# jayleicn/TVRetrieval

Measured on AMD Instinct MI355X. Metric: queries/sec VCMR over 21.8K-video corpus, higher is better.
Workload: dtype bf16

## Files before the change

include/xmlhip.h:

```cpp
#ifndef XMLHIP_H
#define XMLHIP_H

#include <stddef.h>
#include <stdint.h>

#ifdef __cplusplus
extern "C" {
#endif

typedef void* xml_stream_t;

typedef enum { XML_F32 = 0, XML_BF16 = 1, XML_F16 = 2, XML_F16S = 3 } xml_dtype;
#define XML_F16_UNIT_LOG2 14

typedef enum {
  XML_OK = 0,
  XML_ERR_BAD_ARG = -1,
  XML_ERR_UNSUPPORTED = -2,
  XML_ERR_WORKSPACE = -3,
  XML_ERR_LAUNCH = -4
} xml_status;

int xml_abi_version(void);
const char* xml_build_arch(void);
// ... 2 lines not shown
int xml_pack_weights(const float* src, void* dst, int dt, int64_t n, xml_stream_t stream);
int xml_convert(const void* src, int src_dt, void* dst, int dst_dt, int64_t n, xml_stream_t stream);

size_t xml_linear_ln_relu_pos_workspace_bytes(int64_t rows, int d_in, int hidden, int dt);
int xml_linear_ln_relu_pos(const void* x, int x_dt, const float* ln_in_g, const float* ln_in_b,
                           const void* w, const float* b, const void* pos, const float* ln_pos_g,
                           const float* ln_pos_b, void* y, int64_t rows, int seq_len, int d_in,
                           int hidden, int dt, void* ws, size_t ws_bytes, xml_stream_t stream);


size_t xml_attention_block_workspace_bytes(int64_t n, int seq_len, int hidden, int dt);
int xml_attention_block(const void* x, const float* key_mask, const void* wqkv, const float* bqkv,
                        const void* wo, const float* bo, const float* ln_g, const float* ln_b,
                        void* y, int64_t n, int seq_len, int hidden, int n_heads, int dt, void* ws,
                        size_t ws_bytes, xml_stream_t stream);

int xml_attention_core(const void* q, int ldq, const void* k, int ldk, const void* v, int ldv, const float* q_mask,
                       const float* k_mask, void* out, int64_t n, int lq, int lk, int hidden, int n_heads, int dt,
                       xml_stream_t stream);

int xml_pack_plan(const float* mask, int64_t n, int lq, int32_t* cu_seqlens, int32_t* src_row, int32_t* status,
                  xml_stream_t stream);
size_t xml_linear_ln_relu_pos_packed_workspace_bytes(int64_t rows, int d_in, int hidden, int dt);
int xml_linear_ln_relu_pos_packed(const void* x, int x_dt, const int32_t* src_row, int lq, const float* ln_in_g,
                                  const float* ln_in_b, const void* w, const float* b, const void* pos,
                                  const float* ln_pos_g, const float* ln_pos_b, void* y, int64_t rows, int d_in,
                                  int hidden, int dt, void* ws, size_t ws_bytes, xml_stream_t stream);
size_t xml_attention_block_varlen_workspace_bytes(int64_t rows, int hidden, int dt);
int xml_attention_block_varlen(const void* x, const int32_t* cu_seqlens, const void* wqkv, const float* bqkv,
                               const void* wo, const float* bo, const float* ln_g, const float* ln_b, void* y,
// ... 263 lines not shown
```

tvretrieval_amd/_lib.py:

```python
import ctypes
import os
from ctypes import c_char_p, c_float, c_int, c_int32, c_int64, c_size_t, c_void_p

_HERE = os.path.dirname(os.path.abspath(__file__))
LIB_PATH = os.environ.get("XMLHIP_LIB") or os.path.join(_HERE, "csrc", "libxmlhip.so")

XML_F32 = 0
XML_BF16 = 1
XML_F16 = 2
XML_F16S = 3

ABI_VERSION = 6


class XmlHipError(RuntimeError):
    pass


class ConvseDesc(ctypes.Structure):
    _fields_ = [(n, c_int) for n in
                ("nq", "nv", "kpairs", "lpad", "l_ref", "hidden", "n_mod", "merged", "ksize", "softmax", "dt")]


SIGNATURES = {
    "xml_abi_version": (c_int, []),
    "xml_build_arch": (c_char_p, []),
    "xml_status_string": (c_char_p, [c_int]),
    "xml_pack_weights": (c_int, [c_void_p, c_void_p, c_int, c_int64, c_void_p]),
    "xml_convert": (c_int, [c_void_p, c_int, c_void_p, c_int, c_int64, c_void_p]),
    "xml_linear_ln_relu_pos_workspace_bytes": (c_size_t, [c_int64, c_int, c_int, c_int]),
    "xml_linear_ln_relu_pos": (c_int, [c_void_p, c_int, c_void_p, c_void_p, c_void_p, c_void_p, c_void_p, c_void_p,
                                       c_void_p, c_void_p, c_int64, c_int, c_int, c_int, c_int, c_void_p, c_size_t,
                                       c_void_p]),
    "xml_attention_block_workspace_bytes": (c_size_t, [c_int64, c_int, c_int, c_int]),
    "xml_attention_block": (c_int, [c_void_p, c_void_p, c_void_p, c_void_p, c_void_p, c_void_p, c_void_p, c_void_p,
                                    c_void_p, c_int64, c_int, c_int, c_int, c_int, c_void_p, c_size_t, c_void_p]),
    "xml_pack_plan": (c_int, [c_void_p, c_int64, c_int, c_void_p, c_void_p, c_void_p, c_void_p]),
    "xml_linear_ln_relu_pos_packed_workspace_bytes": (c_size_t, [c_int64, c_int, c_int, c_int]),
    "xml_linear_ln_relu_pos_packed": (c_int, [c_void_p, c_int, c_void_p, c_int, c_void_p, c_void_p, c_void_p, c_void_p,
                                              c_void_p, c_void_p, c_void_p, c_void_p, c_int64, c_int, c_int, c_int,
                                              c_void_p, c_size_t, c_void_p]),
    "xml_attention_block_varlen_workspace_bytes": (c_size_t, [c_int64, c_int, c_int]),
    "xml_attention_block_varlen": (c_int, [c_void_p, c_void_p, c_void_p, c_void_p, c_void_p, c_void_p, c_void_p, c_void_p,
                                           c_void_p, c_int64, c_int64, c_int, c_int, c_int, c_int, c_void_p, c_size_t,
                                           c_void_p]),
    "xml_modular_pool_varlen": (c_int, [c_void_p, c_void_p, c_void_p, c_void_p, c_int64, c_int, c_int, c_int, c_int,
                                        c_void_p]),
    "xml_cross_attention_workspace_bytes": (c_size_t, [c_int64, c_int, c_int, c_int, c_int]),
    "xml_cross_attention": (c_int, [c_void_p, c_void_p, c_void_p, c_void_p, c_void_p, c_void_p, c_void_p, c_void_p,
                                    c_void_p, c_void_p, c_void_p, c_int64, c_int, c_int, c_int, c_int, c_int,
                                    c_void_p, c_size_t, c_void_p]),
# ... 198 lines not shown
```

tvretrieval_amd/csrc/attention.hip:

```cpp
#include <type_traits>

#include "gemm.h"
#include "internal.h"

template <typename T> struct ChunkOf { static constexpr int elems = 64 / (int)sizeof(T); };

typedef short xml_v4s __attribute__((ext_vector_type(4)));
__device__ __forceinline__ uint2 lds_read_tr16(const char* p) {
  const xml_v4s r = __builtin_amdgcn_ds_read_tr16_b64_v4i16((__attribute__((address_space(3))) xml_v4s*)p);
  return __builtin_bit_cast(uint2, r);
}

#ifdef XML_DEBUG_VARIANTS
__device__ unsigned long long g_attn_probe[16];
extern "C" int xml_debug_read_attn_probe(unsigned long long* host_out) {
  return hipMemcpyFromSymbol(host_out, HIP_SYMBOL(g_attn_probe), sizeof(unsigned long long) * 16) == hipSuccess ? 0 : -4;
}
#define XML_ATTN_PROBE(i) do { if (abl == 8 && blockIdx.x == 1 && blockIdx.y == 300 && threadIdx.x == 64) g_attn_probe[i] = __builtin_amdgcn_s_memtime(); } while (0)
#else
#define XML_ATTN_PROBE(i) do { } while (0)
#endif

template <typename T, typename OutT, int DH>
__global__ __launch_bounds__(256) void attention_core_kernel(const T* __restrict__ Q, int ldq,
// ... 523 lines not shown
  if (!q || !k || !v || !k_mask || !out) return XML_ERR_BAD_ARG;
  if (dt != XML_F32 && dt != XML_BF16) return XML_ERR_BAD_ARG;
  if (ldq < hidden || ldk < hidden || ldv < hidden || (ldq | ldk | ldv | hidden) % 8) return XML_ERR_UNSUPPORTED;
  return xmli_attention_core(q, ldq, k, ldk, v, ldv, q_mask, k_mask, out, 0, n, lq, lk, hidden, n_heads, dt,
                             (hipStream_t)stream);
}

extern "C" size_t xml_attention_block_workspace_bytes(int64_t n, int seq_len, int hidden, int dt) {
  const size_t rows = (size_t)n * seq_len;
  const size_t pre = align_up(rows * hidden * 4, 256);
  const size_t lnw = xmli_gemm_ln_eligible((int64_t)rows, hidden, hidden, dt) ? xmli_gemm_ln_workspace_bytes((int64_t)rows, hidden) : 0;
  return align_up(rows * 3 * hidden * dt_size(dt), 256) + align_up(rows * hidden * dt_size(dt), 256) +
         (pre > lnw ? pre : lnw) + xmli_gemm_split_ws_bytes((int64_t)rows, hidden, dt);
}

extern "C" int xml_attention_block(const void* x, const float* key_mask, const void* wqkv, const float* bqkv,
                                   const void* wo, const float* bo, const float* ln_g, const float* ln_b, void* y,
                                   int64_t n, int seq_len, int hidden, int n_heads, int dt, void* ws, size_t ws_bytes,
                                   xml_stream_t stream) {
  XML_ENTER();
  if (!x || !key_mask || !wqkv || !bqkv || !wo || !bo || !ln_g || !ln_b || !y || !ws) return XML_ERR_BAD_ARG;
  if (n <= 0 || seq_len <= 0 || !xmli_model_dt_ok(dt)) return XML_ERR_BAD_ARG;
  if (seq_len > 128 || hidden % 8) return XML_ERR_UNSUPPORTED;
  if (ws_bytes < xml_attention_block_workspace_bytes(n, seq_len, hidden, dt)) return XML_ERR_WORKSPACE;
  hipStream_t st = (hipStream_t)stream;
  const int64_t rows = n * seq_len;
  const int adt = xmli_act_dt(dt);
  char* qkv = (char*)ws;
  char* att = qkv + align_up((size_t)rows * 3 * hidden * dt_size(dt), 256);
  char* pre = att + align_up((size_t)rows * hidden * dt_size(dt), 256);
  char* sws = dt == XML_F16S ? (char*)ws + xml_attention_block_workspace_bytes(n, seq_len, hidden, dt) -
                                   xmli_gemm_split_ws_bytes(rows, hidden, dt) : nullptr;
  int rc = xmli_gemm(x, wqkv, bqkv, nullptr, qkv, rows, 3 * hidden, hidden, 0, 0, 1, 0, dt, st, sws);
  if (rc) return rc;
  const size_t es = dt_size(dt);
  rc = xmli_attention_core(qkv, 3 * hidden, qkv + (size_t)hidden * es, 3 * hidden, qkv + (size_t)2 * hidden * es,
                           3 * hidden, nullptr, key_mask, att, 0, n, seq_len, seq_len, hidden, n_heads, adt, st);
  if (rc) return rc;
  if (xmli_gemm_ln_eligible(rows, hidden, hidden, dt) && y != x &&
      xmli_gemm_ln(att, wo, bo, x, ln_g, ln_b, y, rows, hidden, hidden, 0,  2, 1, dt, pre, st) == XML_OK)
    return XML_OK;
  rc = xmli_gemm(att, wo, bo, x, pre, rows, hidden, hidden, 0,  2, 1,  1, dt, st, sws);
  if (rc) return rc;
  return xmli_gemm_ln_tail((const float*)pre, ln_g, ln_b, y, rows, hidden, dt, st);
}

template <typename T, int DH>
static int launch_attn_varlen(const char* qkv, int hidden, const int32_t* cu, void* att, int64_t n, int max_len,
                              int n_heads, int dt, hipStream_t st) {
  const size_t lds_s = attn_small_lds_bytes(max_len, DH, dt);
  if (lds_s > 160 * 1024) return XML_ERR_UNSUPPORTED;
  if (lds_s > 64 * 1024 && !xml_lds_attr_once<attention_core_small_kernel<T, T, DH>>(160 * 1024)) return XML_ERR_LAUNCH;
  const int64_t units = n * n_heads;
  const T* q = (const T*)qkv;
  hipLaunchKernelGGL((attention_core_small_kernel<T, T, DH>), dim3((unsigned)((units + 3) / 4)), dim3(256), lds_s, st, q,
                     3 * hidden, q + hidden, 3 * hidden, q + 2 * hidden, 3 * hidden, (const float*)nullptr,
                     (const float*)nullptr, (T*)att, hidden, max_len, max_len, n_heads, units, sqrtf((float)DH), cu);
  XML_CHECK_LAUNCH();
  return XML_OK;
// ... 430 lines not shown
```

tvretrieval_amd/csrc/gemm256p.hip:

```cpp
#include <type_traits>

#include "common.h"
#include "internal.h"

struct G256pArgs {
  const void* A;
  const void* W;
  const float* bias;
  const void* addend;
  void* out;
  int64_t M, n_tiles;
  int N, K, relu, add_mode, seq_len, tn;
  float* ln_scratch;
  const float* ln_g;
  const float* ln_b;
  float ln_eps;
  int probe;
};

__device__ __forceinline__ void g256p_dma_pair(uint32_t v0, uint32_t v1, const char* sb, uint32_t lds_dst) {
  asm volatile(
      "s_mov_b32 m0, %2\n\ts_nop 0\n\tglobal_load_lds_dwordx4 %0, %3\n\t"
      "s_add_u32 m0, m0, 0x400\n\ts_nop 0\n\tglobal_load_lds_dwordx4 %1, %3"
      :
      : "v"(v0), "v"(v1), "s"(lds_dst), "s"(sb)
      : "memory", "scc");
}
__device__ __forceinline__ void g256p_dma_quad(uint32_t v0, uint32_t v1, uint32_t v2, uint32_t v3, const char* sb,
                                               uint32_t lds_dst) {
  asm volatile(
      "s_mov_b32 m0, %4\n\ts_nop 0\n\tglobal_load_lds_dwordx4 %0, %5\n\t"
      "s_add_u32 m0, m0, 0x400\n\ts_nop 0\n\tglobal_load_lds_dwordx4 %1, %5\n\t"
// ... 36 lines not shown
__device__ __forceinline__ uint4 dpp_u4(const uint4& v) {
  uint4 r;
  r.x = (uint32_t)__builtin_amdgcn_update_dpp(0, (int)v.x, CTRL, 0xf, 0xf, false);
  r.y = (uint32_t)__builtin_amdgcn_update_dpp(0, (int)v.y, CTRL, 0xf, 0xf, false);
  r.z = (uint32_t)__builtin_amdgcn_update_dpp(0, (int)v.z, CTRL, 0xf, 0xf, false);
  r.w = (uint32_t)__builtin_amdgcn_update_dpp(0, (int)v.w, CTRL, 0xf, 0xf, false);
  return r;
}
__device__ __forceinline__ int g256p_lane_now() {
  int l;
  asm volatile("v_mbcnt_lo_u32_b32 %0, -1, 0\n\tv_mbcnt_hi_u32_b32 %0, -1, %0" : "=v"(l));
  return l;
}
__device__ __forceinline__ int g256p_swz(int row) { return (0x78 >> (((row >> 2) & 3) << 1)) & 3; }

template <typename T, typename OutT, typename AddT, bool LNE = false, bool DIRECT = true>
__global__ __launch_bounds__(512) void gemm256p_kernel(G256pArgs a) {
  static_assert(!LNE || DIRECT, "the LayerNorm epilogue works on the DIRECT accumulator layout");
  constexpr int ROWB = 64;
  constexpr int OPER_BYTES = 256 * ROWB;
  constexpr int SLOT_BYTES = 2 * OPER_BYTES;
  constexpr int NSLOT = 4;
  constexpr int RING_BYTES = NSLOT * SLOT_BYTES;
  extern __shared__ __attribute__((aligned(16))) char smem[];

  const int tid = threadIdx.x, lane = tid & 63;
  const int wave = __builtin_amdgcn_readfirstlane(tid >> 6);
  const int wm = wave >> 1, wn = wave & 1;
  const int grp = wave >> 2;
  const int fr = lane & 15, fg = lane >> 4;
  const int xcd = blockIdx.x & 7, loc = blockIdx.x >> 3;
  const int k_bytes = a.K * (int)sizeof(T);
  const int n_slices = k_bytes / ROWB;
// ... 177 lines not shown
    };
    slice_step(faA, faB, std::true_type{});
    slice_step(faB, faA, std::false_type{});
    for (int s2 = 2; s2 < n_slices; s2 += 2) {
      slice_step(faA, faB, std::false_type{});
      slice_step(faB, faA, std::false_type{});
    }

    { const unsigned long long t = G256P_T(); pr[0] += t - pt; pt = t; }
    {
      int64_t mt; int nt;
      tile_mt_nt(c_k, mt, nt);
      const int64_t m0 = mt * 256;
      const int n0 = nt * 256;
      const uint32_t m0_mod = a.add_mode == 1 ? (uint32_t)(m0 % a.seq_len) : 0u;
      const int lane_e = g256p_lane_now();
      const int fr_e = lane_e & 15, fg_e = lane_e >> 4;
      const int tid_e = wave * 64 + lane_e;
      float* patch = reinterpret_cast<float*>(smem + RING_BYTES) + wave * 1024;
      constexpr bool F32O = sizeof(OutT) == 4;
      const int orow = lane_e >> 4;
      const int oc0 = (lane_e & 15) * (F32O ? 4 : 8);
      const int oc1 = F32O ? oc0 + 64 : oc0 + 4;
      const int nc0 = n0 + wn * 128 + oc0, nc1 = n0 + wn * 128 + oc1;
      const bool ok0 = nc0 + 4 <= N, ok1 = nc1 + 4 <= N;
      constexpr int GC = PAIRED ? 8 : 4;
      constexpr int NGRP = 128 / (4 * GC);
      static_assert(GC * sizeof(AddT) <= 16, "addend group wider than one 16-byte load");
      int gcol[DIRECT ? NGRP : 1];
      bool gok[DIRECT ? NGRP : 1];
      int pcol[DIRECT ? NGRP / 2 : 1];
      auto store_rows = [&](int m4, auto& v, int dcol = 0) {
        uint4 pk[NGRP];
#pragma unroll
        for (int q = 0; q < NGRP; ++q) pk[q] = pack16<OutT>(v[q]);
        const bool odd = (fr_e & 1) != 0;
        const int64_t m_even = m0 + wm * 64 + m4 * 16 + (fr_e & ~1);
#pragma unroll
        for (int pq = 0; pq < NGRP / 2; ++pq) {
          const uint4 dn = dpp_u4<0x111>(pk[2 * pq + 1]);
          const uint4 up = dpp_u4<0x101>(pk[2 * pq]);
          const uint4 own_e = pk[2 * pq], own_o = pk[2 * pq + 1];
          const uint4 d_even = make_uint4(odd ? dn.x : own_e.x, odd ? dn.y : own_e.y, odd ? dn.z : own_e.z, odd ? dn.w : own_e.w);
          const uint4 d_odd = make_uint4(odd ? own_o.x : up.x, odd ? own_o.y : up.y, odd ? own_o.z : up.z, odd ? own_o.w : up.w);
          const int col = pcol[pq] + dcol;
          if (col + GC <= N) {
            if (!(a.probe & 8)) {
              typedef unsigned int g_u4 __attribute__((ext_vector_type(4)));
              if (m_even < M && !(a.probe & 4)) __builtin_nontemporal_store(g_u4{d_even.x, d_even.y, d_even.z, d_even.w}, reinterpret_cast<g_u4*>(out + m_even * N + col));
              if (m_even + 1 < M && !(a.probe & 4)) __builtin_nontemporal_store(g_u4{d_odd.x, d_odd.y, d_odd.z, d_odd.w}, reinterpret_cast<g_u4*>(out + (m_even + 1) * N + col));
            } else {
              if (m_even < M && !(a.probe & 4)) st_global16(out + m_even * N + col, d_even);
              if (m_even + 1 < M && !(a.probe & 4)) st_global16(out + (m_even + 1) * N + col, d_odd);
            }
          }
        }
      };
      if constexpr (DIRECT) {
#pragma unroll
        for (int q = 0; q < NGRP; ++q) {
          gcol[q] = n0 + wn * 128 + q * (4 * GC) + fg_e * GC;
          gok[q] = gcol[q] + GC <= N;
        }
#pragma unroll
        for (int pq = 0; pq < NGRP / 2; ++pq) pcol[pq] = n0 + wn * 128 + pq * (8 * GC) + (fr_e & 1) * (4 * GC) + fg_e * GC;
        {
          float4 b4 = make_float4(0.f, 0.f, 0.f, 0.f);
          const int bc = n0 + wn * 128 + (lane_e & 31) * 4;
// ... 255 lines not shown
#ifdef XML_DEBUG_VARIANTS
  if ((a.probe & 1) && blockIdx.x == 0 && lane == 0) {
    pr[5] = __builtin_amdgcn_s_memtime() - pr_t0;
    pr[7] = __builtin_amdgcn_s_memrealtime() - pr_r0;
    for (int i = 0; i < 8; ++i) g_g256p_probe[wave * 8 + i] = pr[i];
    for (int i = 0; i < 64; ++i) g_g256p_steps[wave * 64 + i] = sp[i];
  }
#endif
  };
  if (grp) run(std::true_type{});
  else run(std::false_type{});
  asm volatile("s_waitcnt vmcnt(0)" ::: "memory");
  __builtin_amdgcn_s_barrier();
}

template <typename T, typename OutT, typename AddT, bool LNE = false, bool DIRECT = true>
static int launch_gemm256p(const void* A, const void* W, const float* bias, const void* addend, void* out, int64_t M,
                           int N, int K, int relu, int add_mode, int seq_len, hipStream_t st, const float* ln_g = nullptr,
                           const float* ln_b = nullptr, void* ln_ws = nullptr) {
  G256pArgs a;
  a.A = A; a.W = W; a.bias = bias; a.addend = addend; a.out = out;
  a.M = M; a.N = N; a.K = K; a.relu = relu; a.add_mode = add_mode; a.seq_len = seq_len;
  a.tn = cdiv(N, 256);
  a.n_tiles = (int64_t)cdiv(M, 256) * a.tn;
  a.ln_scratch = (float*)ln_ws; a.ln_g = ln_g; a.ln_b = ln_b; a.ln_eps = 1e-5f;
  a.probe = g_q2c_ablation == 9 ? 1 : g_q2c_ablation == 21 ? 2 : g_q2c_ablation == 22 ? 4 : g_q2c_ablation == 23 ? 6 : g_q2c_ablation == 24 ? 8 : 0;
  const int lds = 4 * 2 * 256 * 64 + 8 * 4096;
#ifdef XML_DEBUG_VARIANTS
  if (!LNE && DIRECT && g_gemm_variant == 3)
    return launch_gemm256p<T, OutT, AddT, false, false>(A, W, bias, addend, out, M, N, K, relu, add_mode, seq_len, st);
#endif
  auto kern = gemm256p_kernel<T, OutT, AddT, LNE, DIRECT>;
  if (!xml_lds_attr_once<gemm256p_kernel<T, OutT, AddT, LNE, DIRECT>>(lds)) return XML_ERR_LAUNCH;
  hipLaunchKernelGGL(kern, dim3(256), dim3(512), lds, st, a);
  XML_CHECK_LAUNCH();
  return XML_OK;
}

static constexpr int64_t LN_FUSED_MIN_ROWS = 2048;

bool xmli_gemm_ln_eligible(int64_t M, int N, int K, int dt) {
  if (dt != XML_F32 && dt != XML_BF16) return false;
  const size_t kb = (size_t)K * dt_size(dt);
  return kb % 128 == 0 && kb >= 256 && N % 256 == 0 && N / 256 <= 3 && M >= LN_FUSED_MIN_ROWS;
}
size_t xmli_gemm_ln_workspace_bytes(int64_t M, int N) {
  (void)M;
  return align_up((size_t)256 * (size_t)(N / 256 > 1 ? N / 256 - 1 : 0) * 256 * 256 * 4 + 256, 256);
}
int xmli_gemm_ln(const void* A, const void* W, const float* bias, const void* addend, const float* ln_g, const float* ln_b,
                 void* y, int64_t M, int N, int K, int relu, int add_mode, int seq_len, int dt, void* ln_ws,
                 hipStream_t st) {
  if (!ln_ws) return XML_ERR_WORKSPACE;
  if (dt == XML_F32)
    return launch_gemm256p<float, float, float, true>(A, W, bias, addend, y, M, N, K, relu, add_mode, seq_len, st, ln_g,
                                                      ln_b, ln_ws);
  return launch_gemm256p<bf16_t, bf16_t, bf16_t, true>(A, W, bias, addend, y, M, N, K, relu, add_mode, seq_len, st, ln_g,
                                                        ln_b, ln_ws);
}

template <typename OutT, int TN>
__global__ __launch_bounds__(64) void ln_lne_order_kernel(const float* __restrict__ pre, const float* __restrict__ ln_g,
                                                           const float* __restrict__ ln_b, OutT* __restrict__ y,
                                                           int64_t rows, int N, float ln_eps) {
#pragma clang fp contract(off)
  constexpr int GC = sizeof(OutT) == 2 ? 8 : 4;
  constexpr int NGRP = 128 / (4 * GC);
  constexpr int LPR = TN == 1 ? 8 : TN == 2 ? 16 : 32;
  const int lane = threadIdx.x & 63;
  const int sub = lane & (LPR - 1);
  const int base = lane - sub;
  const int64_t row = ((int64_t)blockIdx.x * 64 + threadIdx.x) / LPR;
  if (row >= rows || sub >= 8 * TN) return;
  const int seg = sub >> 2, fg = sub & 3;
  const int c0 = (seg >> 1) * 256 + (seg & 1) * 128 + fg * GC;
  const float* pr = pre + row * N;
  float v[NGRP][GC], gv[NGRP][GC], bv[NGRP][GC];
#pragma unroll
  for (int q = 0; q < NGRP; ++q)
#pragma unroll
    for (int e = 0; e < GC; e += 4) {
      const float4 f = *reinterpret_cast<const float4*>(pr + c0 + q * (4 * GC) + e);
      const float4 g4 = *reinterpret_cast<const float4*>(ln_g + c0 + q * (4 * GC) + e);
      const float4 b4 = *reinterpret_cast<const float4*>(ln_b + c0 + q * (4 * GC) + e);
      v[q][e] = f.x; v[q][e + 1] = f.y; v[q][e + 2] = f.z; v[q][e + 3] = f.w;
      gv[q][e] = g4.x; gv[q][e + 1] = g4.y; gv[q][e + 2] = g4.z; gv[q][e + 3] = g4.w;
      bv[q][e] = b4.x; bv[q][e + 1] = b4.y; bv[q][e + 2] = b4.z; bv[q][e + 3] = b4.w;
    }
#pragma unroll
  for (int q = 0; q < NGRP; ++q)
#pragma unroll
// ... 29 lines not shown
  float m2 = 0.f;
#pragma unroll
  for (int t = 0; t < TN; ++t) {
    const float d0 = __builtin_fmaf(pv[t].x, 1.0f / 128.0f, -mean), d1 = __builtin_fmaf(pv[t].z, 1.0f / 128.0f, -mean);
    float u = __builtin_fmaf(d0, 128.0f * d0, pv[t].y);
    u = pv[t].w + u;
    u = __builtin_fmaf(d1, 128.0f * d1, u);
    m2 = u + m2;
  }
  const float rstd = 1.0f / sqrtf(m2 / (float)N + ln_eps);
#pragma unroll
  for (int q = 0; q < NGRP; ++q) {
    float o[GC];
#pragma unroll
    for (int e = 0; e < GC; ++e) o[e] = __builtin_fmaf((v[q][e] - mean) * rstd, gv[q][e], bv[q][e]);
    st_global16(y + row * N + c0 + q * (4 * GC), pack16<OutT>(o));
  }
}

int xmli_gemm_ln_tail(const float* pre, const float* ln_g, const float* ln_b, void* y, int64_t M, int N, int dt,
                      hipStream_t st) {
  const int tn = N / 256;
  if ((dt != XML_F32 && dt != XML_BF16) || N % 256 || tn < 1 || tn > 3 || M <= 0)
    return xmli_add_layernorm(pre, XML_F32, nullptr, ln_g, ln_b, y, M, N, N, xmli_act_dt(dt), st);
  const int lpr = tn == 1 ? 8 : tn == 2 ? 16 : 32;
  const dim3 grid((unsigned)cdiv(M * lpr, (int64_t)64)), blk(64);
#define XML_LNT(OT, TN)                                                                                                 \
  hipLaunchKernelGGL((ln_lne_order_kernel<OT, TN>), grid, blk, 0, st, pre, ln_g, ln_b, (OT*)y, M, N, 1e-5f)
  if (dt == XML_F32) {
    if (tn == 1) XML_LNT(float, 1); else if (tn == 2) XML_LNT(float, 2); else XML_LNT(float, 3);
  } else {
    if (tn == 1) XML_LNT(bf16_t, 1); else if (tn == 2) XML_LNT(bf16_t, 2); else XML_LNT(bf16_t, 3);
  }
#undef XML_LNT
  XML_CHECK_LAUNCH();
  return XML_OK;
}

bool xmli_gemm256p_eligible(int64_t M, int N, int K, int dt) {
  const size_t kb = (size_t)K * dt_size(dt);
  return kb % 128 == 0 && kb >= 256 && N >= 128 && N % 8 == 0 && (int64_t)cdiv(M, 256) * cdiv(N, 256) >= 3072;
}

// ... 9 lines not shown
```

tvretrieval_amd/csrc/internal.h:

```cpp
#pragma once
#include "common.h"

int xmli_gemm(const void* A, const void* W, const float* bias, const void* addend, void* out, int64_t M, int N,
              int K, int relu, int add_mode, int seq_len, int out_f32, int dt, hipStream_t st, void* split_ws = nullptr);
size_t xmli_gemm_split_ws_bytes(int64_t M, int K, int dt);
static inline int xmli_act_dt(int dt) { return dt == XML_F16S ? XML_F32 : dt; }
static inline bool xmli_model_dt_ok(int dt) { return dt == XML_F32 || dt == XML_BF16 || dt == XML_F16S; }
bool xmli_gemm_ln_eligible(int64_t M, int N, int K, int dt);
size_t xmli_gemm_ln_workspace_bytes(int64_t M, int N);
int xmli_gemm_ln(const void* A, const void* W, const float* bias, const void* addend, const float* ln_g, const float* ln_b,
                 void* y, int64_t M, int N, int K, int relu, int add_mode, int seq_len, int dt, void* ln_ws,
                 hipStream_t st);
int xmli_gemm_ln_tail(const float* pre, const float* ln_g, const float* ln_b, void* y, int64_t M, int N, int dt,
                      hipStream_t st);
int xmli_add_layernorm(const void* a, int a_dt, const void* b, const float* g, const float* beta, void* y,
                       int64_t rows, int d, int ld_out, int dt, hipStream_t st);
int xmli_attention_core(const void* q, int ldq, const void* k, int ldk, const void* v, int ldv,
                        const float* q_mask, const float* k_mask, void* out, int out_f32, int64_t n, int lq, int lk,
                        int hidden, int n_heads, int dt, hipStream_t st);
int xmli_modular_pool_bwd_vec(const void* enc, const float* mask, const float* w_m, const void* dout, void* denc, float* dw_m,
                              int64_t n, int lq, int hidden, int n_mod, int dt, hipStream_t st);
```

tvretrieval_amd/inference.py:

```python
import numpy as np
import torch

from . import ops as hip_ops


def _round_up(x, m):
    return (x + m - 1) // m * m


class CorpusIndex(object):

    def __init__(self, modalities, feat1n, feat2, mask, l_ref, video_offset=0, n_total=None):
        self.modalities = list(modalities)
        self.feat1n, self.feat2, self.mask = feat1n, feat2, mask
        self.l_ref = int(l_ref)
        self.lpad = int(feat2[self.modalities[0]].shape[1])
        self.n_videos = int(feat2[self.modalities[0]].shape[0])
        self.video_offset = int(video_offset)
        self.n_total = int(n_total if n_total is not None else self.n_videos)
        self.feat2_all = self.mask_all = None
        self.exact = None
        self.vlen = self.vlen_all = None
        self.ragged = False

# ... 98 lines not shown
        self.n_videos, self.l_ref, self.lpad = int(n_videos), int(l_ref), index_lpad(l_ref, model, ops)
        self.f1 = {m: torch.zeros((self.n_videos, self.lpad, h), dtype=dt, device=dev) for m in mods}
        self.f2 = {m: torch.zeros((self.n_videos, self.lpad, h), dtype=dt, device=dev) for m in mods}
        self.mk = {m: torch.zeros((self.n_videos, self.lpad), dtype=torch.float32, device=dev) for m in mods}
        self.tiles = {}
        if tiles and hasattr(ops, "q2c_tiled_numel") and self.lpad == 128 and dt in (torch.float32, torch.bfloat16):
            n = ops.q2c_tiled_numel(self.n_videos * self.lpad, h, dt)
            if n:
                self.tiles = {m: torch.zeros(n, dtype=dt, device=dev) for m in mods}

    def nbytes(self):
        return sum(t.numel() * t.element_size() for d in (self.f1, self.f2, self.mk, self.tiles) for t in d.values())


def build_corpus_index(model, context_batches, ops=hip_ops, keep_raw=False, video_offset=0, n_total=None,
                        l_ref=None, n_videos=None, exact_filter=False, storage=None):
    mods = [n for n, u in (("video", model.use_video), ("sub", model.use_sub)) if u]
    if storage is not None:
        assert l_ref is None or int(l_ref) == storage.l_ref
        assert n_videos is None or int(n_videos) == storage.n_videos
        l_ref, n_videos = storage.l_ref, storage.n_videos
    if n_videos is not None and l_ref is not None:
        return _build_corpus_index_prealloc(model, context_batches, ops, keep_raw, video_offset, n_total, int(l_ref),
                                            int(n_videos), mods, exact_filter, storage)
    parts = {m: dict(f1=[], f2=[], mk=[]) for m in mods}
    for video_feat, video_mask, sub_feat, sub_mask in context_batches:
        v1, v2, s1, s2 = model.encode_context(video_feat, video_mask, sub_feat, sub_mask)
        if "video" in parts:
            parts["video"]["f1"].append(v1), parts["video"]["f2"].append(v2), parts["video"]["mk"].append(video_mask.float())
        if "sub" in parts:
            parts["sub"]["f1"].append(s1), parts["sub"]["f2"].append(s2), parts["sub"]["mk"].append(sub_mask.float())
    batch_max = max(t.shape[1] for t in parts[mods[0]]["f2"])
    l_ref = batch_max if l_ref is None else int(l_ref)
    assert l_ref >= batch_max
    lpad = index_lpad(l_ref, model, ops)

    def cat(tensors):
        n = sum(t.shape[0] for t in tensors)
        out = tensors[0].new_zeros((n, lpad) + tuple(tensors[0].shape[2:]))
# ... 22 lines not shown
            raw[m] = f1
    idx = CorpusIndex(mods, feat1n, feat2, mask, l_ref, video_offset, n_total)
    if getattr(ops, "RAGGED_ROWS", False):
        idx.set_valid_lengths()
    idx.raw_feat1 = raw
    if exact_filter:
        idx.exact = _make_exact_filter(ex_f32, ex_ec, exact_mode_of(model, ops))
    return idx


def _make_exact_filter(ex_f32, ex_ec, mode):
    return ExactFilter(ex_f32, ex_ec, n_candidates=128 if (mode == "f16s" and EXACT_F16S_FILTER == "f16") else 256, mode=mode)


def _build_corpus_index_prealloc(model, context_batches, ops, keep_raw, video_offset, n_total, l_ref, n_videos, mods,
                                 exact_filter=False, storage=None):
    lpad = index_lpad(l_ref, model, ops)
    f1, f2, mk = {}, {}, {}
    if storage is not None:
        f1, f2, mk = dict(storage.f1), dict(storage.f2), dict(storage.mk)
    r = 0
    for video_feat, video_mask, sub_feat, sub_mask in context_batches:
        outs = [None, None, None, None]
        direct = bool(f1) and getattr(ops, "ENCODE_INTO_INDEX", False)
        if direct:
            for i, (m, feat) in enumerate((("video", video_feat), ("sub", sub_feat))):
                b = feat.shape[0] if feat is not None else 0
                if m in mods and feat is not None and feat.shape[1] == lpad and r + b <= n_videos:
                    outs[2 * i], outs[2 * i + 1] = f1[m][r:r + b], f2[m][r:r + b]
                elif m in mods:
                    direct = False
        if direct:
            v1, v2, s1, s2 = model.encode_context(video_feat, video_mask, sub_feat, sub_mask, outs=tuple(outs))
        else:
            v1, v2, s1, s2 = model.encode_context(video_feat, video_mask, sub_feat, sub_mask)
        for m, a1, a2, am in (("video", v1, v2, video_mask), ("sub", s1, s2, sub_mask)):
            if m not in mods:
                continue
            if m not in f1:
                f1[m] = a1.new_zeros((n_videos, lpad, a1.shape[2]))
                f2[m] = a2.new_zeros((n_videos, lpad, a2.shape[2]))
                mk[m] = torch.zeros((n_videos, lpad), dtype=torch.float32, device=a1.device)
            b, lb = a1.shape[0], a1.shape[1]
            assert r + b <= n_videos and lb <= l_ref
            if not direct:
                f1[m][r:r + b, :lb] = a1
                f2[m][r:r + b, :lb] = a2
            mk[m][r:r + b, :lb] = am.float()
        r += v1.shape[0] if v1 is not None else s1.shape[0]
    assert r == n_videos, "n_videos=%d but the batches held %d" % (n_videos, r)
    plan = ops.q2c_pack_plan([mk[m] for m in mods]) if (hasattr(ops, "q2c_pack_plan") and lpad == 128) else None
    feat1n, raw, ex_f32, ex_ec = {}, {}, {}, {}
    for m in mods:
        if exact_filter:
            feat1n[m], ex_f32[m], ex_ec[m] = _exact_filter_operands(f1[m], mk[m], plan, ops, exact_mode_of(model, ops))
            if exact_mode_of(model, ops) == "f16s":
                f2[m] = ops.split_f16_rows(f2[m])
        else:
            tile_buf = storage.tiles.get(m) if (storage is not None and plan is None) else None
            kw = dict(out=tile_buf) if tile_buf is not None else {}
            feat1n[m] = ops.pack_q2c_corpus(f1[m], mk[m], plan, normalize=True, **kw) if hasattr(ops, "pack_q2c_corpus") \
# ... 1148 lines not shown
```

tvretrieval_amd/ops.py:

```python
import collections
import ctypes

import os

import numpy as np

import torch

from . import _lib
from ._lib import XML_BF16, XML_F32, ConvseDesc, check

class _SplitF16(object):

    def __repr__(self):
        return "tvretrieval_amd.ops.F16S"


F16S = _SplitF16()
_DT = {torch.float32: XML_F32, torch.bfloat16: XML_BF16, torch.float16: _lib.XML_F16, F16S: _lib.XML_F16S}
F16_UNIT_LOG2 = 14


def act_dtype(dtype):
    return torch.float32 if dtype is F16S else dtype
# ... 125 lines not shown
    if v < 0:
        check(v, what)
    return v


ENCODE_INTO_INDEX = True


def _req_w(w, name, x):
    _req(w, name)
    if not (w.dtype == x.dtype or (w.dtype is F16S and x.dtype == torch.float32)):
        raise _lib.XmlHipError("%s: weight dtype %s does not go with activations of dtype %s" % (name, w.dtype, x.dtype))
    return w


def attention_block(x, key_mask, wqkv, bqkv, wo, bo, ln_g, ln_b, n_heads, out=None):
    _req(x, "x"); _req(key_mask, "key_mask", torch.float32); _req_w(wqkv, "wqkv", x); _req_w(wo, "wo", x)
    for t, nm in ((bqkv, "bqkv"), (bo, "bo"), (ln_g, "ln_g"), (ln_b, "ln_b")):
        _req(t, nm, torch.float32)
    n, seq_len, hidden = x.shape
    lib = _lib.load()
    dt = dt_of(wqkv)
    if out is None:
        y = torch.empty_like(x)
    else:
        _req(out, "out", x.dtype)
        assert out.shape == x.shape and out.data_ptr() != x.data_ptr()
        y = out
    ws = _workspace(lib.xml_attention_block_workspace_bytes(n, seq_len, hidden, dt), x.device)
    check(lib.xml_attention_block(_p(x), _p(key_mask), _p(wqkv), _p(bqkv), _p(wo), _p(bo), _p(ln_g), _p(ln_b), _p(y),
                                  n, seq_len, hidden, n_heads, dt, _p(ws), ws.numel(), _stream()),
          "xml_attention_block")
    return y


def attention_core(q, k, v, q_mask, k_mask, n_heads):
    _req(q, "q"); _req(k, "k", q.dtype); _req(v, "v", q.dtype); _req(k_mask, "k_mask", torch.float32)
    if q_mask is not None:
        _req(q_mask, "q_mask", torch.float32)
    n, lq, hidden = q.shape
    lk = k.shape[1]
    assert k.shape == v.shape and k.shape[0] == n and k.shape[2] == hidden
    out = torch.empty((n, lq, hidden), dtype=q.dtype, device=q.device)
    check(_lib.load().xml_attention_core(_p(q), hidden, _p(k), hidden, _p(v), hidden, _p(q_mask), _p(k_mask), _p(out), n, lq,
                                         lk, hidden, int(n_heads), dt_of(q), _stream()), "xml_attention_core")
    return out

# ... 889 lines not shown
```

Before: 146,700.

## Write attention-block output directly into padded corpus index via strided rows

Adds a sequence-strided output mode to the attention block, covering both the GEMM+LayerNorm epilogue kernel and the LN tail kernel, so encoder output can land straight in a slice of the preallocated padded index tensors even when the batch length is shorter than the index padding. The Python index builder now infers n_videos up front, preallocates the index (using torch.empty when every batch already matches the padding), and passes strided views into encode_context. This is meant to remove the intermediate output tensors and the copy into the index, plus the zero-fill. The cost is extra per-row address arithmetic (divide/modulo) in the epilogue and more complex control flow in the builder.

After: 146,700 (median of 2 runs). Within noise of the previous version (-0.0%).

```diff
diff --git a/include/xmlhip.h b/include/xmlhip.h
--- a/include/xmlhip.h
+++ b/include/xmlhip.h
@@ -40,6 +40,11 @@
                         const void* wo, const float* bo, const float* ln_g, const float* ln_b,
                         void* y, int64_t n, int seq_len, int hidden, int n_heads, int dt, void* ws,
                         size_t ws_bytes, xml_stream_t stream);
+int xml_attention_block_to_ok(int hidden, int dt);
+int xml_attention_block_to(const void* x, const float* key_mask, const void* wqkv, const float* bqkv,
+                           const void* wo, const float* bo, const float* ln_g, const float* ln_b,
+                           void* y, int64_t y_seq_stride, int64_t n, int seq_len, int hidden, int n_heads, int dt,
+                           void* ws, size_t ws_bytes, xml_stream_t stream);
 
 int xml_attention_core(const void* q, int ldq, const void* k, int ldk, const void* v, int ldv, const float* q_mask,
                        const float* k_mask, void* out, int64_t n, int lq, int lk, int hidden, int n_heads, int dt,
diff --git a/tvretrieval_amd/_lib.py b/tvretrieval_amd/_lib.py
--- a/tvretrieval_amd/_lib.py
+++ b/tvretrieval_amd/_lib.py
@@ -35,6 +35,9 @@
     "xml_attention_block_workspace_bytes": (c_size_t, [c_int64, c_int, c_int, c_int]),
     "xml_attention_block": (c_int, [c_void_p, c_void_p, c_void_p, c_void_p, c_void_p, c_void_p, c_void_p, c_void_p,
                                     c_void_p, c_int64, c_int, c_int, c_int, c_int, c_void_p, c_size_t, c_void_p]),
+    "xml_attention_block_to_ok": (c_int, [c_int, c_int]),
+    "xml_attention_block_to": (c_int, [c_void_p, c_void_p, c_void_p, c_void_p, c_void_p, c_void_p, c_void_p, c_void_p,
+                                       c_void_p, c_int64, c_int64, c_int, c_int, c_int, c_int, c_void_p, c_size_t, c_void_p]),
     "xml_pack_plan": (c_int, [c_void_p, c_int64, c_int, c_void_p, c_void_p, c_void_p, c_void_p]),
     "xml_linear_ln_relu_pos_packed_workspace_bytes": (c_size_t, [c_int64, c_int, c_int, c_int]),
     "xml_linear_ln_relu_pos_packed": (c_int, [c_void_p, c_int, c_void_p, c_int, c_void_p, c_void_p, c_void_p, c_void_p,
diff --git a/tvretrieval_amd/csrc/attention.hip b/tvretrieval_amd/csrc/attention.hip
--- a/tvretrieval_amd/csrc/attention.hip
+++ b/tvretrieval_amd/csrc/attention.hip
@@ -561,14 +561,17 @@
          (pre > lnw ? pre : lnw) + xmli_gemm_split_ws_bytes((int64_t)rows, hidden, dt);
 }
 
-extern "C" int xml_attention_block(const void* x, const float* key_mask, const void* wqkv, const float* bqkv,
-                                   const void* wo, const float* bo, const float* ln_g, const float* ln_b, void* y,
-                                   int64_t n, int seq_len, int hidden, int n_heads, int dt, void* ws, size_t ws_bytes,
-                                   xml_stream_t stream) {
-  XML_ENTER();
+static int attention_block_impl(const void* x, const float* key_mask, const void* wqkv, const float* bqkv,
+                                const void* wo, const float* bo, const float* ln_g, const float* ln_b, void* y,
+                                int64_t y_seq_stride, int64_t n, int seq_len, int hidden, int n_heads, int dt, void* ws,
+                                size_t ws_bytes, xml_stream_t stream) {
   if (!x || !key_mask || !wqkv || !bqkv || !wo || !bo || !ln_g || !ln_b || !y || !ws) return XML_ERR_BAD_ARG;
   if (n <= 0 || seq_len <= 0 || !xmli_model_dt_ok(dt)) return XML_ERR_BAD_ARG;
   if (seq_len > 128 || hidden % 8) return XML_ERR_UNSUPPORTED;
+  if (y_seq_stride < (int64_t)seq_len * hidden) return XML_ERR_BAD_ARG;
+  const int y_seq_len = y_seq_stride == (int64_t)seq_len * hidden ? 0 : seq_len;
+  if (y_seq_len && !xml_attention_block_to_ok(hidden, dt)) return XML_ERR_UNSUPPORTED;
+  if (y_seq_len && (y_seq_stride % 8 || y == x)) return XML_ERR_UNSUPPORTED;
   if (ws_bytes < xml_attention_block_workspace_bytes(n, seq_len, hidden, dt)) return XML_ERR_WORKSPACE;
   hipStream_t st = (hipStream_t)stream;
   const int64_t rows = n * seq_len;
@@ -585,11 +588,34 @@
                            3 * hidden, nullptr, key_mask, att, 0, n, seq_len, seq_len, hidden, n_heads, adt, st);
   if (rc) return rc;
   if (xmli_gemm_ln_eligible(rows, hidden, hidden, dt) && y != x &&
-      xmli_gemm_ln(att, wo, bo, x, ln_g, ln_b, y, rows, hidden, hidden, 0,  2, 1, dt, pre, st) == XML_OK)
+      xmli_gemm_ln(att, wo, bo, x, ln_g, ln_b, y, rows, hidden, hidden, 0,  2, 1, dt, pre, st, y_seq_stride,
+                   y_seq_len) == XML_OK)
     return XML_OK;
   rc = xmli_gemm(att, wo, bo, x, pre, rows, hidden, hidden, 0,  2, 1,  1, dt, st, sws);
   if (rc) return rc;
-  return xmli_gemm_ln_tail((const float*)pre, ln_g, ln_b, y, rows, hidden, dt, st);
+  return xmli_gemm_ln_tail((const float*)pre, ln_g, ln_b, y, rows, hidden, dt, st, y_seq_stride, y_seq_len);
+}
+
+extern "C" int xml_attention_block(const void* x, const float* key_mask, const void* wqkv, const float* bqkv,
+                                   const void* wo, const float* bo, const float* ln_g, const float* ln_b, void* y,
+                                   int64_t n, int seq_len, int hidden, int n_heads, int dt, void* ws, size_t ws_bytes,
+                                   xml_stream_t stream) {
+  XML_ENTER();
+  return attention_block_impl(x, key_mask, wqkv, bqkv, wo, bo, ln_g, ln_b, y, (int64_t)seq_len * hidden, n, seq_len, hidden,
+                              n_heads, dt, ws, ws_bytes, stream);
+}
+
+extern "C" int xml_attention_block_to_ok(int hidden, int dt) {
+  return (dt == XML_F32 || dt == XML_BF16) && hidden > 0 && hidden % 256 == 0 && hidden / 256 <= 3;
+}
+
+extern "C" int xml_attention_block_to(const void* x, const float* key_mask, const void* wqkv, const float* bqkv,
+                                      const void* wo, const float* bo, const float* ln_g, const float* ln_b, void* y,
+                                      int64_t y_seq_stride, int64_t n, int seq_len, int hidden, int n_heads, int dt, void* ws,
+                                      size_t ws_bytes, xml_stream_t stream) {
+  XML_ENTER();
+  return attention_block_impl(x, key_mask, wqkv, bqkv, wo, bo, ln_g, ln_b, y, y_seq_stride, n, seq_len, hidden, n_heads, dt,
+                              ws, ws_bytes, stream);
 }
 
 template <typename T, int DH>
diff --git a/tvretrieval_amd/csrc/gemm256p.hip b/tvretrieval_amd/csrc/gemm256p.hip
--- a/tvretrieval_amd/csrc/gemm256p.hip
+++ b/tvretrieval_amd/csrc/gemm256p.hip
@@ -16,6 +16,8 @@
   const float* ln_b;
   float ln_eps;
   int probe;
+  int64_t out_seq_stride;
+  int out_seq_len;
 };
 
 __device__ __forceinline__ void g256p_dma_pair(uint32_t v0, uint32_t v1, const char* sb, uint32_t lds_dst) {
@@ -82,9 +84,10 @@
 }
 __device__ __forceinline__ int g256p_swz(int row) { return (0x78 >> (((row >> 2) & 3) << 1)) & 3; }
 
-template <typename T, typename OutT, typename AddT, bool LNE = false, bool DIRECT = true>
+template <typename T, typename OutT, typename AddT, bool LNE = false, bool DIRECT = true, bool OSEQ = false>
 __global__ __launch_bounds__(512) void gemm256p_kernel(G256pArgs a) {
   static_assert(!LNE || DIRECT, "the LayerNorm epilogue works on the DIRECT accumulator layout");
+  static_assert(!OSEQ || LNE, "sequence-strided output rows: LayerNorm-epilogue kernels only");
   constexpr int ROWB = 64;
   constexpr int OPER_BYTES = 256 * ROWB;
   constexpr int SLOT_BYTES = 2 * OPER_BYTES;
@@ -292,6 +295,12 @@
       const int64_t m0 = mt * 256;
       const int n0 = nt * 256;
       const uint32_t m0_mod = a.add_mode == 1 ? (uint32_t)(m0 % a.seq_len) : 0u;
+      int64_t o_seq0 = 0;
+      uint32_t o_row0 = 0;
+      if constexpr (OSEQ) {
+        o_seq0 = m0 / a.out_seq_len;
+        o_row0 = (uint32_t)(m0 - o_seq0 * a.out_seq_len);
+      }
       const int lane_e = g256p_lane_now();
       const int fr_e = lane_e & 15, fg_e = lane_e >> 4;
       const int tid_e = wave * 64 + lane_e;
@@ -314,6 +323,15 @@
         for (int q = 0; q < NGRP; ++q) pk[q] = pack16<OutT>(v[q]);
         const bool odd = (fr_e & 1) != 0;
         const int64_t m_even = m0 + wm * 64 + m4 * 16 + (fr_e & ~1);
+        OutT* o_even = nullptr;
+        OutT* o_odd = nullptr;
+        if constexpr (OSEQ) {
+          const uint32_t sl = (uint32_t)a.out_seq_len;
+          const uint32_t u0 = o_row0 + (uint32_t)(wm * 64 + m4 * 16 + (fr_e & ~1)), u1 = u0 + 1;
+          const uint32_t d0 = u0 / sl, d1 = u1 / sl;
+          o_even = out + (o_seq0 + d0) * a.out_seq_stride + (int64_t)(u0 - d0 * sl) * N;
+          o_odd = out + (o_seq0 + d1) * a.out_seq_stride + (int64_t)(u1 - d1 * sl) * N;
+        }
 #pragma unroll
         for (int pq = 0; pq < NGRP / 2; ++pq) {
           const uint4 dn = dpp_u4<0x111>(pk[2 * pq + 1]);
@@ -325,11 +343,11 @@
           if (col + GC <= N) {
             if (!(a.probe & 8)) {
               typedef unsigned int g_u4 __attribute__((ext_vector_type(4)));
-              if (m_even < M && !(a.probe & 4)) __builtin_nontemporal_store(g_u4{d_even.x, d_even.y, d_even.z, d_even.w}, reinterpret_cast<g_u4*>(out + m_even * N + col));
-              if (m_even + 1 < M && !(a.probe & 4)) __builtin_nontemporal_store(g_u4{d_odd.x, d_odd.y, d_odd.z, d_odd.w}, reinterpret_cast<g_u4*>(out + (m_even + 1) * N + col));
+              if (m_even < M && !(a.probe & 4)) __builtin_nontemporal_store(g_u4{d_even.x, d_even.y, d_even.z, d_even.w}, reinterpret_cast<g_u4*>(OSEQ ? o_even + col : out + m_even * N + col));
+              if (m_even + 1 < M && !(a.probe & 4)) __builtin_nontemporal_store(g_u4{d_odd.x, d_odd.y, d_odd.z, d_odd.w}, reinterpret_cast<g_u4*>(OSEQ ? o_odd + col : out + (m_even + 1) * N + col));
             } else {
-              if (m_even < M && !(a.probe & 4)) st_global16(out + m_even * N + col, d_even);
-              if (m_even + 1 < M && !(a.probe & 4)) st_global16(out + (m_even + 1) * N + col, d_odd);
+              if (m_even < M && !(a.probe & 4)) st_global16(OSEQ ? o_even + col : out + m_even * N + col, d_even);
+              if (m_even + 1 < M && !(a.probe & 4)) st_global16(OSEQ ? o_odd + col : out + (m_even + 1) * N + col, d_odd);
             }
           }
         }
@@ -615,24 +633,26 @@
   __builtin_amdgcn_s_barrier();
 }
 
-template <typename T, typename OutT, typename AddT, bool LNE = false, bool DIRECT = true>
+template <typename T, typename OutT, typename AddT, bool LNE = false, bool DIRECT = true, bool OSEQ = false>
 static int launch_gemm256p(const void* A, const void* W, const float* bias, const void* addend, void* out, int64_t M,
                            int N, int K, int relu, int add_mode, int seq_len, hipStream_t st, const float* ln_g = nullptr,
-                           const float* ln_b = nullptr, void* ln_ws = nullptr) {
+                           const float* ln_b = nullptr, void* ln_ws = nullptr, int64_t out_seq_stride = 0,
+                           int out_seq_len = 0) {
   G256pArgs a;
   a.A = A; a.W = W; a.bias = bias; a.addend = addend; a.out = out;
   a.M = M; a.N = N; a.K = K; a.relu = relu; a.add_mode = add_mode; a.seq_len = seq_len;
   a.tn = cdiv(N, 256);
   a.n_tiles = (int64_t)cdiv(M, 256) * a.tn;
   a.ln_scratch = (float*)ln_ws; a.ln_g = ln_g; a.ln_b = ln_b; a.ln_eps = 1e-5f;
+  a.out_seq_stride = out_seq_stride; a.out_seq_len = out_seq_len;
   a.probe = g_q2c_ablation == 9 ? 1 : g_q2c_ablation == 21 ? 2 : g_q2c_ablation == 22 ? 4 : g_q2c_ablation == 23 ? 6 : g_q2c_ablation == 24 ? 8 : 0;
   const int lds = 4 * 2 * 256 * 64 + 8 * 4096;
 #ifdef XML_DEBUG_VARIANTS
   if (!LNE && DIRECT && g_gemm_variant == 3)
     return launch_gemm256p<T, OutT, AddT, false, false>(A, W, bias, addend, out, M, N, K, relu, add_mode, seq_len, st);
 #endif
-  auto kern = gemm256p_kernel<T, OutT, AddT, LNE, DIRECT>;
-  if (!xml_lds_attr_once<gemm256p_kernel<T, OutT, AddT, LNE, DIRECT>>(lds)) return XML_ERR_LAUNCH;
+  auto kern = gemm256p_kernel<T, OutT, AddT, LNE, DIRECT, OSEQ>;
+  if (!xml_lds_attr_once<gemm256p_kernel<T, OutT, AddT, LNE, DIRECT, OSEQ>>(lds)) return XML_ERR_LAUNCH;
   hipLaunchKernelGGL(kern, dim3(256), dim3(512), lds, st, a);
   XML_CHECK_LAUNCH();
   return XML_OK;
@@ -651,8 +671,16 @@
 }
 int xmli_gemm_ln(const void* A, const void* W, const float* bias, const void* addend, const float* ln_g, const float* ln_b,
                  void* y, int64_t M, int N, int K, int relu, int add_mode, int seq_len, int dt, void* ln_ws,
-                 hipStream_t st) {
+                 hipStream_t st, int64_t y_seq_stride, int y_seq_len) {
   if (!ln_ws) return XML_ERR_WORKSPACE;
+  if (y_seq_len > 0 && y_seq_stride != (int64_t)y_seq_len * N) {
+    if (y_seq_stride < (int64_t)y_seq_len * N) return XML_ERR_BAD_ARG;
+    if (dt == XML_F32)
+      return launch_gemm256p<float, float, float, true, true, true>(A, W, bias, addend, y, M, N, K, relu, add_mode, seq_len,
+                                                                    st, ln_g, ln_b, ln_ws, y_seq_stride, y_seq_len);
+    return launch_gemm256p<bf16_t, bf16_t, bf16_t, true, true, true>(A, W, bias, addend, y, M, N, K, relu, add_mode, seq_len,
+                                                                      st, ln_g, ln_b, ln_ws, y_seq_stride, y_seq_len);
+  }
   if (dt == XML_F32)
     return launch_gemm256p<float, float, float, true>(A, W, bias, addend, y, M, N, K, relu, add_mode, seq_len, st, ln_g,
                                                       ln_b, ln_ws);
@@ -660,10 +688,11 @@
                                                         ln_b, ln_ws);
 }
 
-template <typename OutT, int TN>
+template <typename OutT, int TN, bool OSEQ = false>
 __global__ __launch_bounds__(64) void ln_lne_order_kernel(const float* __restrict__ pre, const float* __restrict__ ln_g,
                                                            const float* __restrict__ ln_b, OutT* __restrict__ y,
-                                                           int64_t rows, int N, float ln_eps) {
+                                                           int64_t rows, int N, float ln_eps, int64_t y_seq_stride,
+                                                           int y_seq_len) {
 #pragma clang fp contract(off)
   constexpr int GC = sizeof(OutT) == 2 ? 8 : 4;
   constexpr int NGRP = 128 / (4 * GC);
@@ -676,6 +705,8 @@
   const int seg = sub >> 2, fg = sub & 3;
   const int c0 = (seg >> 1) * 256 + (seg & 1) * 128 + fg * GC;
   const float* pr = pre + row * N;
+  OutT* yr = y + row * N;
+  if constexpr (OSEQ) yr = y + (row / y_seq_len) * y_seq_stride + (row % y_seq_len) * (int64_t)N;
   float v[NGRP][GC], gv[NGRP][GC], bv[NGRP][GC];
 #pragma unroll
   for (int q = 0; q < NGRP; ++q)
@@ -735,19 +766,30 @@
     float o[GC];
 #pragma unroll
     for (int e = 0; e < GC; ++e) o[e] = __builtin_fmaf((v[q][e] - mean) * rstd, gv[q][e], bv[q][e]);
-    st_global16(y + row * N + c0 + q * (4 * GC), pack16<OutT>(o));
+    st_global16(yr + c0 + q * (4 * GC), pack16<OutT>(o));
   }
 }
 
 int xmli_gemm_ln_tail(const float* pre, const float* ln_g, const float* ln_b, void* y, int64_t M, int N, int dt,
-                      hipStream_t st) {
+                      hipStream_t st, int64_t y_seq_stride, int y_seq_len) {
   const int tn = N / 256;
-  if ((dt != XML_F32 && dt != XML_BF16) || N % 256 || tn < 1 || tn > 3 || M <= 0)
+  if (y_seq_len > 0 && y_seq_stride == (int64_t)y_seq_len * N) y_seq_len = 0;
+  if ((dt != XML_F32 && dt != XML_BF16) || N % 256 || tn < 1 || tn > 3 || M <= 0) {
+    if (y_seq_len > 0) return XML_ERR_UNSUPPORTED;
     return xmli_add_layernorm(pre, XML_F32, nullptr, ln_g, ln_b, y, M, N, N, xmli_act_dt(dt), st);
+  }
+  if (y_seq_len > 0 && y_seq_stride < (int64_t)y_seq_len * N) return XML_ERR_BAD_ARG;
   const int lpr = tn == 1 ? 8 : tn == 2 ? 16 : 32;
   const dim3 grid((unsigned)cdiv(M * lpr, (int64_t)64)), blk(64);
 #define XML_LNT(OT, TN)                                                                                                 \
-  hipLaunchKernelGGL((ln_lne_order_kernel<OT, TN>), grid, blk, 0, st, pre, ln_g, ln_b, (OT*)y, M, N, 1e-5f)
+  do {                                                                                                                  \
+    if (y_seq_len > 0)                                                                                                  \
+      hipLaunchKernelGGL((ln_lne_order_kernel<OT, TN, true>), grid, blk, 0, st, pre, ln_g, ln_b, (OT*)y, M, N, 1e-5f,   \
+                         y_seq_stride, y_seq_len);                                                                      \
+    else                                                                                                                \
+      hipLaunchKernelGGL((ln_lne_order_kernel<OT, TN, false>), grid, blk, 0, st, pre, ln_g, ln_b, (OT*)y, M, N, 1e-5f,  \
+                         y_seq_stride, y_seq_len);                                                                      \
+  } while (0)
   if (dt == XML_F32) {
     if (tn == 1) XML_LNT(float, 1); else if (tn == 2) XML_LNT(float, 2); else XML_LNT(float, 3);
   } else {
diff --git a/tvretrieval_amd/csrc/internal.h b/tvretrieval_amd/csrc/internal.h
--- a/tvretrieval_amd/csrc/internal.h
+++ b/tvretrieval_amd/csrc/internal.h
@@ -10,9 +10,9 @@
 size_t xmli_gemm_ln_workspace_bytes(int64_t M, int N);
 int xmli_gemm_ln(const void* A, const void* W, const float* bias, const void* addend, const float* ln_g, const float* ln_b,
                  void* y, int64_t M, int N, int K, int relu, int add_mode, int seq_len, int dt, void* ln_ws,
-                 hipStream_t st);
+                 hipStream_t st, int64_t y_seq_stride = 0, int y_seq_len = 0);
 int xmli_gemm_ln_tail(const float* pre, const float* ln_g, const float* ln_b, void* y, int64_t M, int N, int dt,
-                      hipStream_t st);
+                      hipStream_t st, int64_t y_seq_stride = 0, int y_seq_len = 0);
 int xmli_add_layernorm(const void* a, int a_dt, const void* b, const float* g, const float* beta, void* y,
                        int64_t rows, int d, int ld_out, int dt, hipStream_t st);
 int xmli_attention_core(const void* q, int ldq, const void* k, int ldk, const void* v, int ldv,
diff --git a/tvretrieval_amd/inference.py b/tvretrieval_amd/inference.py
--- a/tvretrieval_amd/inference.py
+++ b/tvretrieval_amd/inference.py
@@ -136,15 +136,22 @@
 
 
 def build_corpus_index(model, context_batches, ops=hip_ops, keep_raw=False, video_offset=0, n_total=None,
-                        l_ref=None, n_videos=None, exact_filter=False, storage=None):
+                        l_ref=None, n_videos=None, exact_filter=False, storage=None, direct=True):
     mods = [n for n, u in (("video", model.use_video), ("sub", model.use_sub)) if u]
     if storage is not None:
         assert l_ref is None or int(l_ref) == storage.l_ref
         assert n_videos is None or int(n_videos) == storage.n_videos
         l_ref, n_videos = storage.l_ref, storage.n_videos
+    if direct and n_videos is None and l_ref is not None and isinstance(context_batches, (list, tuple)) and len(context_batches):
+        n_videos = sum((b[0] if b[0] is not None else b[2]).shape[0] for b in context_batches)
+        lpad_ = index_lpad(int(l_ref), model, ops)
+        shapes = [t.shape for b in context_batches for t in (b[0], b[2]) if t is not None]
+        return _build_corpus_index_prealloc(model, context_batches, ops, keep_raw, video_offset, n_total, int(l_ref),
+                                            int(n_videos), mods, exact_filter, storage, direct,
+                                            zero_fill=not all(sh[1] == lpad_ for sh in shapes))
     if n_videos is not None and l_ref is not None:
         return _build_corpus_index_prealloc(model, context_batches, ops, keep_raw, video_offset, n_total, int(l_ref),
-                                            int(n_videos), mods, exact_filter, storage)
+                                            int(n_videos), mods, exact_filter, storage, direct)
     parts = {m: dict(f1=[], f2=[], mk=[]) for m in mods}
     for video_feat, video_mask, sub_feat, sub_mask in context_batches:
         v1, v2, s1, s2 = model.encode_context(video_feat, video_mask, sub_feat, sub_mask)
@@ -197,22 +204,38 @@
 
 
 def _build_corpus_index_prealloc(model, context_batches, ops, keep_raw, video_offset, n_total, l_ref, n_videos, mods,
-                                 exact_filter=False, storage=None):
+                                 exact_filter=False, storage=None, direct=True, zero_fill=True):
     lpad = index_lpad(l_ref, model, ops)
     f1, f2, mk = {}, {}, {}
     if storage is not None:
         f1, f2, mk = dict(storage.f1), dict(storage.f2), dict(storage.mk)
+    into_index = direct and getattr(ops, "ENCODE_INTO_INDEX", False)
     r = 0
     for video_feat, video_mask, sub_feat, sub_mask in context_batches:
+        if into_index and not f1:
+            feat0 = video_feat if video_feat is not None else sub_feat
+            dt0, h0 = getattr(model, "act_dtype", model.compute_dtype), model.config.hidden_size
+            new = torch.zeros if zero_fill else torch.empty
+            for m in mods:
+                f1[m] = new((n_videos, lpad, h0), dtype=dt0, device=feat0.device)
+                f2[m] = new((n_videos, lpad, h0), dtype=dt0, device=feat0.device)
+                mk[m] = new((n_videos, lpad), dtype=torch.float32, device=feat0.device)
         outs = [None, None, None, None]
-        direct = bool(f1) and getattr(ops, "ENCODE_INTO_INDEX", False)
+        direct = bool(f1) and into_index
+        direct1 = direct
         if direct:
             for i, (m, feat) in enumerate((("video", video_feat), ("sub", sub_feat))):
-                b = feat.shape[0] if feat is not None else 0
-                if m in mods and feat is not None and feat.shape[1] == lpad and r + b <= n_videos:
+                b, lb = (feat.shape[0], feat.shape[1]) if feat is not None else (0, 0)
+                if m in mods and feat is not None and r + b <= n_videos and \
+                        (lb == lpad or (lb < lpad and ops.attention_block_strided_ok(f1[m].shape[2], f1[m].dtype))):
                     outs[2 * i], outs[2 * i + 1] = f1[m][r:r + b], f2[m][r:r + b]
+                    if lb != lpad:
+                        outs[2 * i], outs[2 * i + 1] = outs[2 * i][:, :lb], outs[2 * i + 1][:, :lb]
+                    direct1 = direct1 and lb == lpad
                 elif m in mods:
                     direct = False
+        if direct and not direct1:
+            outs[0] = outs[2] = None
         if direct:
             v1, v2, s1, s2 = model.encode_context(video_feat, video_mask, sub_feat, sub_mask, outs=tuple(outs))
         else:
@@ -225,9 +248,10 @@
                 f2[m] = a2.new_zeros((n_videos, lpad, a2.shape[2]))
                 mk[m] = torch.zeros((n_videos, lpad), dtype=torch.float32, device=a1.device)
             b, lb = a1.shape[0], a1.shape[1]
-            assert r + b <= n_videos and lb <= l_ref
+            assert r + b <= n_videos and lb <= l_ref and (zero_fill or lb == lpad)
+            if not (direct and direct1):
+                f1[m][r:r + b, :lb] = a1
             if not direct:
-                f1[m][r:r + b, :lb] = a1
                 f2[m][r:r + b, :lb] = a2
             mk[m][r:r + b, :lb] = am.float()
         r += v1.shape[0] if v1 is not None else s1.shape[0]
diff --git a/tvretrieval_amd/ops.py b/tvretrieval_amd/ops.py
--- a/tvretrieval_amd/ops.py
+++ b/tvretrieval_amd/ops.py
@@ -163,6 +163,10 @@
     return w
 
 
+def attention_block_strided_ok(hidden, dtype):
+    return dtype in _DT and bool(_lib.load().xml_attention_block_to_ok(int(hidden), _DT[dtype]))
+
+
 def attention_block(x, key_mask, wqkv, bqkv, wo, bo, ln_g, ln_b, n_heads, out=None):
     _req(x, "x"); _req(key_mask, "key_mask", torch.float32); _req_w(wqkv, "wqkv", x); _req_w(wo, "wo", x)
     for t, nm in ((bqkv, "bqkv"), (bo, "bo"), (ln_g, "ln_g"), (ln_b, "ln_b")):
@@ -170,16 +174,23 @@
     n, seq_len, hidden = x.shape
     lib = _lib.load()
     dt = dt_of(wqkv)
+    seq_stride = seq_len * hidden
     if out is None:
         y = torch.empty_like(x)
     else:
-        _req(out, "out", x.dtype)
-        assert out.shape == x.shape and out.data_ptr() != x.data_ptr()
+        if not (isinstance(out, torch.Tensor) and out.is_cuda and out.dtype == x.dtype and out.shape == x.shape):
+            raise _lib.XmlHipError("out: expected a GPU tensor of x's shape and dtype")
+        assert out.data_ptr() != x.data_ptr()
+        if not out.is_contiguous():
+            if out.stride(2) != 1 or out.stride(1) != hidden or (n > 1 and out.stride(0) < seq_stride):
+                raise _lib.XmlHipError("out: rows must be dense and sequences must not overlap (strides %s)" % (out.stride(),))
+            if n > 1:
+                seq_stride = out.stride(0)
         y = out
     ws = _workspace(lib.xml_attention_block_workspace_bytes(n, seq_len, hidden, dt), x.device)
-    check(lib.xml_attention_block(_p(x), _p(key_mask), _p(wqkv), _p(bqkv), _p(wo), _p(bo), _p(ln_g), _p(ln_b), _p(y),
-                                  n, seq_len, hidden, n_heads, dt, _p(ws), ws.numel(), _stream()),
-          "xml_attention_block")
+    check(lib.xml_attention_block_to(_p(x), _p(key_mask), _p(wqkv), _p(bqkv), _p(wo), _p(bo), _p(ln_g), _p(ln_b), _p(y),
+                                     seq_stride, n, seq_len, hidden, n_heads, dt, _p(ws), ws.numel(), _stream()),
+          "xml_attention_block_to")
     return y
 
 
```
